# brade31919/radar_depth

Measured on AMD Instinct MI355X. Metric: training samples/sec, resnet18_latefusion b=16 450x800 rgbd, 1/2/4/8 MI355X, higher is better.
Workload: dtype f32

## Files before the change

include/radar_depth_hip.h:

```cpp
#ifndef RADAR_DEPTH_HIP_H
#define RADAR_DEPTH_HIP_H

#include <stdint.h>

#ifdef __cplusplus
extern "C" {
#endif

#define RD_OK 0
#define RD_EINVAL (-1)
#define RD_ELAUNCH (-2)

#define RD_MAX_TAPS 25
#define RD_MAX_PHASES 4

#define RD_ACT_NONE 0
#define RD_ACT_RELU 1
#define RD_ACT_LEAKY02 2

const char* rd_last_error(void);
int rd_abi_version(void);
int rd_device_info(int* n_cu, char* name, int name_len);

typedef struct {
    int32_t n_taps;
    int32_t out_off_h, out_off_w;
    int32_t lh, lw;
    int32_t dh_min, dh_max, dw_min, dw_max;
    int32_t tile_begin;
    int8_t dh[RD_MAX_TAPS];
    int8_t dw[RD_MAX_TAPS];
    int16_t widx[RD_MAX_TAPS];
} RdPhase;

typedef struct {
    int32_t N;
    int32_t Hi, Wi, Cin, ldi;
    int32_t Ho, Wo, Cout, ldo;
    int32_t in_stride, out_stride;
    int32_t n_phases;
    RdPhase phase[RD_MAX_PHASES];
} RdConvDesc;

int rd_gconv(const RdConvDesc* d, const float* in, const float* w_packed, float* out,
             const float* addend, int32_t ld_add, float* stat_partial, void* stream);
int rd_gconv_stat_tiles(const RdConvDesc* d);
int64_t rd_gconv_workspace_floats(const RdConvDesc* d);
int rd_gconv_stat_tiles_ws(const RdConvDesc* d);
int rd_gconv_ws(const RdConvDesc* d, const float* in, const float* w_packed, float* out,
                const float* addend, int32_t ld_add, float* stat_partial, float* ws, void* stream);
int rd_gconv_bnbwd_supported(const RdConvDesc* d);
int rd_gconv_bnbwd(const RdConvDesc* d, const float* dout, const float* w_packed, float* dx, const float* bn_x, int32_t ld_x,
                   const float* bn_mean, const float* bn_scale, const float* bn_shift, int32_t act, float* red_partial, float* ws,
                   void* stream);
int rd_gconv_fused(const RdConvDesc* d, const float* in, const float* w_packed, float* out, const float* bias,
                   int32_t act, int32_t act_cols, const float* addend, int32_t ld_add, float* ws, void* stream);
int rd_gconv_bf16(const RdConvDesc* d, const float* in, const void* w_packed_bf16, float* out, const float* bias,
                  int32_t act, int32_t act_cols, const float* addend, int32_t ld_add, float* stat_partial, void* stream);
int rd_gconv_bf16_stat_tiles(const RdConvDesc* d);
int rd_gconv_bf16_plan_info(const RdConvDesc* d, int32_t* out);
int rd_gconv_bf16_stat_tiles_t(int32_t dtype, const RdConvDesc* d);
int rd_gconv_bf16_plan_info_t(int32_t dtype, const RdConvDesc* d, int32_t* out);
int rd_gconv_bf16p_plan_all(int32_t on);
int rd_gconv_bf16_trace_read(unsigned long long* host, int n_wg);
int rd_gconv_split_supported(const RdConvDesc* d);
int rd_gconv_split_plan_all(int on);
int rd_gconv_split(const RdConvDesc* d, const float* in, const void* w_split, int64_t piece_elems, float* out, const float* bias,
                   int32_t act, int32_t act_cols, const float* addend, int32_t ld_add, float* stat_partial, void* stream);
int rd_gconv_split_stat_tiles(const RdConvDesc* d);
int rd_gconv_split_plan_info(const RdConvDesc* d, int32_t* out);
int rd_gemm_taps_split_supported(const RdConvDesc* d);
int rd_gemm_taps_split_preferred(const RdConvDesc* d);
int rd_gemm_taps_split_stat_tiles(const RdConvDesc* d);
int rd_gemm_taps_split_plan_info(const RdConvDesc* d, int32_t* out);
int rd_gemm_taps_split(const RdConvDesc* d, const float* in, const void* w_split, int64_t piece_elems, float* out, const float* bias,
                       int32_t act, int32_t act_cols, const float* addend, int32_t ld_add, float* stat_partial, void* stream);
int rd_split_pieces(const float* x, int32_t ldx, int64_t M, int32_t C, void* pieces, int64_t piece_elems, void* stream);
int rd_gconv_split_bnbwd_supported(const RdConvDesc* d, int32_t pre);
int rd_gconv_split_bnbwd(const RdConvDesc* d, const float* in, const void* w_split, int64_t piece_elems, float* out, const float* bn_x,
                         int32_t bn_ld, const float* mean, const float* scale, const float* shift, int32_t bn_act, float* red_partial, void* stream);
int rd_gconv_split_pre_bnbwd(const RdConvDesc* d, const void* in_pieces, int64_t in_piece_elems, const void* w_split, int64_t piece_elems,
                             float* out, const float* bn_x, int32_t bn_ld, const float* mean, const float* scale, const float* shift,
                             int32_t bn_act, float* red_partial, void* stream);
int rd_gconv_split_pre_supported(const RdConvDesc* d);
int rd_gconv_split_pre_preferred(const RdConvDesc* d);
int rd_gconv_split_pre(const RdConvDesc* d, const void* in_pieces, int64_t in_piece_elems, const void* w_split, int64_t piece_elems, float* out,
                       const float* bias, int32_t act, int32_t act_cols, const float* addend, int32_t ld_add, float* stat_partial, void* stream);
int rd_gconv_split_pre_stat_tiles(const RdConvDesc* d);
int rd_gconv_split_pre_plan_info(const RdConvDesc* d, int32_t* out);
int rd_gconv_split_slot_map(const RdConvDesc* d, int32_t pre, int32_t phase, int32_t* out, int32_t* slots, int32_t n_slots);
int rd_gconv_split_trace_read(unsigned long long* host, int n_wg);
int rd_wgrad_split_supported(const RdConvDesc* d);
int64_t rd_wgrad_split_workspace_floats(const RdConvDesc* d);
int rd_wgrad_split(const RdConvDesc* d, const float* in, const float* dout, float* slabs, void* stream);
int rd_wgrad_split_reduce(const RdConvDesc* d, const float* slabs, float* grad_oihw, int32_t O, int32_t I, int32_t KH, int32_t KW,
                          int32_t co_off, int32_t accumulate, void* stream);
int rd_wgrad_split_plan_info(const RdConvDesc* d, int32_t* out);
int rd_wgrad_split_pre_supported(const RdConvDesc* d);
int rd_wgrad_split_pre(const RdConvDesc* d, const void* x_pieces, int64_t x_piece_elems, const void* dy_pieces, int64_t dy_piece_elems,
                       float* slabs, void* stream);
int rd_gconv_plan_info(const RdConvDesc* d, int32_t* out);
int rd_gconv_occupancy(const RdConvDesc* d);
int rd_gconv_trace_read(unsigned long long* host, int n_wg);

int64_t rd_wgrad_workspace_floats(const RdConvDesc* d);
int rd_wgrad(const RdConvDesc* d, const float* in, const float* dout, float* slabs, void* stream);
int rd_wgrad_reduce(const RdConvDesc* d, const float* slabs, float* grad_oihw, int32_t O, int32_t I,
                    int32_t KH, int32_t KW, int32_t co_off, int32_t accumulate, void* stream);
int rd_wgrad_plan_info(const RdConvDesc* d, int32_t* out);

int rd_pack_weights(const float* w_oihw, float* packed, int32_t O, int32_t I, int32_t KH, int32_t KW,
                    int32_t ldc, int32_t co_off, int32_t rows_total, int32_t transpose, void* stream);

typedef struct {
    const float* slabs;
    float* tmp;
    float* grad;
    int64_t E;
    int32_t n_splits, J, S, Cin, Cout, O, I, co_off, accumulate;
    int32_t first_block1, n_blocks1, first_block2, n_blocks2;
    int32_t pad_;
} RdReduceJob;
int rd_wgrad_reduce_job(const RdConvDesc* d, int32_t bf16_kernel, const float* slabs, float* grad_oihw, int32_t O, int32_t I,
                        int32_t KH, int32_t KW, int32_t co_off, int32_t accumulate, RdReduceJob* job);
int rd_wgrad_reduce_batched(const RdReduceJob* jobs_dev, const int32_t* block_job1_dev, int32_t n_blocks1,
                            const int32_t* block_job2_dev, int32_t n_blocks2, void* stream);

int rd_wgrad_bf16_supported(const RdConvDesc* d);
int64_t rd_wgrad_bf16_workspace_floats(const RdConvDesc* d);
int rd_wgrad_bf16(const RdConvDesc* d, const float* in, const float* dout, float* slabs, void* stream);
int rd_wgrad_bf16_reduce(const RdConvDesc* d, const float* slabs, float* grad_oihw, int32_t O, int32_t I, int32_t KH,
                         int32_t KW, int32_t co_off, int32_t accumulate, void* stream);
int rd_wgrad_bf16_plan_info(const RdConvDesc* d, int32_t* out);
int rd_wgrad_bf16_trace_read(unsigned long long* host, int n_wg);

int rd_pack_weights_bf16(const float* w_oihw, void* packed_bf16, int32_t O, int32_t I, int32_t KH, int32_t KW,
                         int32_t ldc, int32_t co_off, int32_t rows_total, int32_t transpose, void* stream);

int rd_pack_chunk(void);
int rd_pack_weights_batched(const void* jobs_dev, const int32_t* block_job_dev, int32_t n_blocks, void* stream);

int rd_stem_fwd(const float* const* planes, const int64_t* strides, int32_t Cin, int32_t N, int32_t H,
                int32_t W, const float* w_packed, int32_t Cout, float* out, float* stat_partial,
                void* stream);
int rd_stem_stat_tiles(int32_t N, int32_t H, int32_t W);
int rd_stem_fwd_bf16(const float* const* planes, const int64_t* strides, int32_t Cin, int32_t N, int32_t H,
                     int32_t W, const float* w_packed, int32_t Cout, float* out, float* stat_partial,
                     void* stream);
int rd_stem_fwd_split(const float* const* planes, const int64_t* strides, int32_t Cin, int32_t N, int32_t H,
                      int32_t W, const float* w_packed, int32_t Cout, float* out, float* stat_partial,
                      void* stream);
int rd_conv16_split_supported(const RdConvDesc* d);
int rd_conv16_split(const RdConvDesc* d, const float* in, const float* w_packed, float* out, const float* addend, int32_t ld_add,
                    float* stat_partial, void* stream);
int64_t rd_stem_wgrad_workspace_floats(int32_t N, int32_t H, int32_t W, int32_t Cin, int32_t Cout);
int rd_stem_wgrad(const float* const* planes, const int64_t* strides, int32_t Cin, int32_t N, int32_t H,
                  int32_t W, const float* dout, int32_t Cout, float* grad_oihw, float* ws, void* stream);
int rd_stem_wgrad_split_supported(int32_t Cin, int32_t Cout);
int rd_stem_wgrad_split_t(int32_t dtype, const float* const* planes, const int64_t* strides, int32_t Cin, int32_t N, int32_t H,
                          int32_t W, const void* dout, int32_t Cout, float* grad_oihw, float* ws, void* stream);
int rd_stem_wgrad_split_bn_t(int32_t dtype, const float* const* planes, const int64_t* strides, int32_t Cin, int32_t N, int32_t H,
                             int32_t W, const void* g, const void* x, const float* red_partial, int32_t n_tiles, const float* gamma,
                             const float* mean, const float* invstd, float* dgamma, float* dbeta, float* coef_ws, int32_t Cout,
                             float* grad_oihw, float* ws, void* stream);
int rd_stem_dgrad_channel(const float* dout, const float* w_packed, int32_t N, int32_t H, int32_t W,
                          int32_t Cin, int32_t ci, int32_t Cout, float* dx, void* stream);

int rd_bn_finalize(const float* stat_partial, int32_t n_tiles, int32_t ld, int32_t c0, int32_t C, int64_t count,
                   const float* gamma, const float* beta, float eps, float momentum,
                   float* running_mean, float* running_var, int64_t* num_batches_tracked,
                   float* mean, float* invstd, float* scale, float* shift, void* stream);
int rd_bn_eval_coeffs(int32_t C, const float* gamma, const float* beta, const float* running_mean,
                      const float* running_var, float eps, float* scale, float* shift, void* stream);
int rd_bn_eval_coeffs_batched(const void* jobs_dev, int32_t n_jobs, float eps, void* stream);
int rd_bn_stats(const float* x, int64_t M, int32_t C, int32_t ldx, float* stat_partial, int32_t* n_tiles,
                void* stream);
int rd_bn_stats_tiles(int64_t M);
int rd_bn_act(const float* x1, int32_t ldx1, const float* scale1, const float* shift1,
              const float* x2, int32_t ldx2, const float* scale2, const float* shift2,
              float* y, int32_t ldy, int64_t M, int32_t C, int32_t act, void* stream);
int rd_bn_bwd_reduce(const float* dy, int32_t lddy, const float* y, int32_t ldy,
                     const float* x1, int32_t ldx1, const float* mean1,
                     const float* x2, int32_t ldx2, const float* mean2,
                     float* g, int32_t ldg, int64_t M, int32_t C, int32_t act,
                     float* red_partial, void* stream);
int rd_bn_bwd_reduce_x(const float* dy, int32_t lddy, const float* x1, int32_t ldx1, const float* mean1,
                       const float* scale1, const float* shift1, float* g, int32_t ldg, int64_t M, int32_t C,
                       int32_t act, float* red_partial, void* stream);
int rd_bn_bwd_tiles(int64_t M, int32_t C);
int rd_bn_bwd_apply(const float* g, int32_t ldg, const float* x, int32_t ldx, const float* red_partial,
                    int32_t n_tiles, int32_t which, const float* gamma, const float* mean,
                    const float* invstd, float* dgamma, float* dbeta, float* coef_ws ,
                    float* dx, int32_t lddx, int64_t M, int32_t C, void* stream);
int rd_bn_bwd_apply_x(const float* dy, int32_t lddy, const float* x, int32_t ldx, const float* red_partial, int32_t n_tiles,
                      const float* gamma, const float* mean, const float* invstd, const float* scale, const float* shift,
                      int32_t act, float* dgamma, float* dbeta, float* coef_ws, float* dx, int32_t lddx, int64_t M, int32_t C,
                      void* stream);
int rd_bn_bwd_reduce_x2(const float* dy, int32_t lddy, const float* x1, int32_t ldx1, const float* mean1, const float* scale1,
                        const float* shift1, const float* x2, int32_t ldx2, const float* mean2, const float* scale2,
                        const float* shift2, int64_t M, int32_t C, int32_t act, float* red_partial, void* stream);
int rd_bn_bwd_apply_x2(const float* dy, int32_t lddy, const float* x1, int32_t ldx1, const float* x2, int32_t ldx2,
                       const float* red_partial, int32_t n_tiles, const float* gamma1, const float* mean1, const float* invstd1,
                       const float* scale1, const float* shift1, const float* gamma2, const float* mean2, const float* invstd2,
                       const float* scale2, const float* shift2, int32_t act, float* dgamma1, float* dbeta1, float* dgamma2,
                       float* dbeta2, float* coef_ws6, float* dx1, int32_t lddx1, float* dx2, int32_t lddx2, int64_t M,
                       int32_t C, void* stream);

int rd_bnact_maxpool_fwd(const float* x, const float* scale, const float* shift, int32_t act,
                         int32_t N, int32_t H, int32_t W, int32_t C, float* y, int32_t ldy,
                         uint8_t* idx, void* stream);
int rd_bnact_maxpool_bwd(const float* dy, int32_t lddy, const uint8_t* idx, const float* x,
                         const float* scale, const float* shift, int32_t act, int32_t N, int32_t H,
                         int32_t W, int32_t C, float* g, void* stream);
int rd_bnact_maxpool_bwd_tiles(int32_t N, int32_t H, int32_t W, int32_t C);
int rd_bnact_maxpool_bwd_stats(const float* dy, int32_t lddy, const uint8_t* idx, const float* x, const float* scale,
                               const float* shift, int32_t act, int32_t N, int32_t H, int32_t W, int32_t C, float* g,
                               const float* mean, float* red_partial, void* stream);

int rd_head_conv_fwd(const float* x, int32_t ldx, const float* w_oihw, int32_t N, int32_t H, int32_t W,
                     int32_t C, float* d, void* stream);
int rd_head_conv_bwd(const float* x, int32_t ldx, const float* w_oihw, const float* dd, int32_t N,
                     int32_t H, int32_t W, int32_t C, float* dx, int32_t lddx, float* dw_oihw,
                     float* ws, void* stream);
int64_t rd_head_conv_bwd_workspace_floats(int32_t N, int32_t H, int32_t W, int32_t C);
int rd_bilinear_fwd(const float* d, int32_t N, int32_t Hs, int32_t Ws, float* out, int32_t Ho, int32_t Wo,
                    void* stream);
int rd_bilinear_bwd(const float* dout, int32_t N, int32_t Ho, int32_t Wo, float* dd, int32_t Hs, int32_t Ws,
                    void* stream);

int rd_masked_l1_sums(const float* pred, const float* target, int64_t n, float* ws, double* sums, void* stream);
int rd_loss_tiles(int64_t n);
int rd_masked_l1_bwd(const float* pred, const float* target, int64_t n, const double* sums,
                     const float* coef, float* dpred, int32_t accumulate, void* stream);
int rd_masked_l2_sums(const float* pred, const float* target, int64_t n, float* ws, double* sums, void* stream);
int rd_masked_l2_bwd(const float* pred, const float* target, int64_t n, const double* sums,
                     const float* coef, float* dpred, int32_t accumulate, void* stream);
int rd_depth_metrics(const float* output, const float* target, int64_t n, float* ws, double* sums, void* stream);
int rd_masked_l1_sums_metrics(const float* pred, const float* target, int64_t n, float* ws, double* sums,
                              double* msums, void* stream);
int rd_masked_l2_sums_metrics(const float* pred, const float* target, int64_t n, float* ws, double* sums,
                              double* msums, void* stream);
int64_t rd_depth_metrics_frames_workspace_floats(int32_t frames, int64_t hw);
int rd_depth_metrics_frames(const float* output, const float* target, int32_t frames, int64_t hw, float* ws,
                            double* sums, void* stream);
int rd_meter_update(const double* sums, int32_t rows, const double* weights, const int32_t* groups,
                    int32_t n_groups, double* meter, double* last, void* stream);
int64_t rd_smooth_workspace_floats(int32_t N, int32_t H, int32_t W);
int rd_smooth_fwd(const float* pred, const float* image, int32_t N, int32_t C, int32_t H, int32_t W,
                  float* ws, double* out, void* stream);
int rd_smooth_bwd(int32_t N, int32_t H, int32_t W, const float* ws, const float* coef, float* dpred,
// ... 163 lines not shown
```

radar_depth_amd/csrc/wgrad_split.hip:

```cpp
#include <math.h>
#include <stdlib.h>

#include <mutex>
#include <string>
#include <unordered_map>

#include "common.h"

namespace rd {

int launch_slab_reduce(const float* slabs, int n_splits, int64_t E, float* tmp, float* grad_oihw, int S, int Cin, int Cout,
                       int O, int I, int co_off, int accumulate, hipStream_t s);

typedef __bf16 wsbf16x8 __attribute__((ext_vector_type(8)));
typedef short wss16x4 __attribute__((ext_vector_type(4)));
typedef unsigned int wsu32x4 __attribute__((ext_vector_type(4)));
typedef float wsf32x2 __attribute__((ext_vector_type(2)));
typedef __bf16 wsbf16x2 __attribute__((ext_vector_type(2)));

constexpr unsigned WS_OOB = 0x80000000u;
template <int R_, int TW_>
struct WsGeo {
    static constexpr int R = R_, TW = TW_;
    static constexpr int XW = TW + 2, XH = R + 2;
    static constexpr int XPIX = XW * XH, YPIX = R * TW;
    static constexpr int XPLANE = ((XPIX * 64 + 255) / 256) * 256;
    static constexpr int YPLANE = YPIX * 64;
    static constexpr int XBYTES = 3 * 2 * XPLANE;
    static constexpr int YBYTES = 3 * 2 * YPLANE;
    static constexpr int BUF = XBYTES + YBYTES;
    static constexpr int XUNITS = XPIX * 8;
    static constexpr int XUNITS_PAD = ((XUNITS + 63) / 64) * 64;
    static constexpr int UNITS = XUNITS_PAD + YPIX * 8;
    static constexpr int UPT = (UNITS + 255) / 256;
    static_assert(YPIX == 64 && TW % 16 == 0, "a tile is 64 pixels in 16-pixel reduction steps");
    static constexpr int XP16 = ((XPIX * 32 + 127) / 256) * 256 + 128;
    static constexpr int YP16 = ((YPIX * 32 + 127) / 256) * 256 + 128;
    static constexpr int XBYTES_P = 3 * 4 * XP16;
    static constexpr int YBYTES_P = 3 * 4 * YP16;
    static constexpr int BUF_P = XBYTES_P + YBYTES_P;
    static constexpr int XSEG = (XW + 31) / 32, YSEG = (TW + 31) / 32;
    static constexpr int XU_P = 3 * 4 * XH * XSEG;
    static constexpr int YU_P = 3 * 4 * R * YSEG;
};
typedef WsGeo<2, 32> WsWide;
typedef WsGeo<4, 16> WsTall;

struct WsArgs {
    const float* x;
    const float* dy;
    float* slabs;
    int N, Hi, Wi, Cin, ldi, Ho, Wo, Cout, ldo;
    int tiles_h, tiles_w, total_tiles, tiles_per_split, n_splits, n_cib, n_cob;
    int dh0, dw0;
    int OS, off_h, off_w;
    int lh, lw;
    int S;
    int widx[9];
    const unsigned short* xp;
    const unsigned short* yp;
    long long xplane, yplane;
    long long xm, ym;
    int dbg;
};

__device__ __forceinline__ unsigned ws_cvt_pk(float a, float b) {
    wsf32x2 v;
    v[0] = a; v[1] = b;
    return __builtin_bit_cast(unsigned, __builtin_convertvector(v, wsbf16x2));
}
__device__ __forceinline__ void ws_split8(const float4 v0, const float4 v1, wsu32x4& w0, wsu32x4& w1, wsu32x4& w2) {
    const float x[8] = {v0.x, v0.y, v0.z, v0.w, v1.x, v1.y, v1.z, v1.w};
#pragma unroll
    for (int i = 0; i < 4; ++i) {
        float a = x[2 * i], b = x[2 * i + 1];
        const unsigned u0 = ws_cvt_pk(a, b);
        a -= __uint_as_float(u0 << 16);
        b -= __uint_as_float(u0 & 0xffff0000u);
        const unsigned u1 = ws_cvt_pk(a, b);
        a -= __uint_as_float(u1 << 16);
        b -= __uint_as_float(u1 & 0xffff0000u);
        w0[i] = u0;
        w1[i] = u1;
        w2[i] = ws_cvt_pk(a, b);
    }
}

template <int PITCH = 64>
__device__ __forceinline__ wsbf16x8 ws_frag(unsigned base, int off) {
    typedef __attribute__((address_space(3))) wss16x4* lp;
    const wss16x4 lo = __builtin_amdgcn_ds_read_tr16_b64_v4i16(reinterpret_cast<lp>(base + off));
    const wss16x4 hi = __builtin_amdgcn_ds_read_tr16_b64_v4i16(reinterpret_cast<lp>(base + off + 4 * PITCH));
    typedef short s16x8 __attribute__((ext_vector_type(8)));
    s16x8 r;
    r[0] = lo[0]; r[1] = lo[1]; r[2] = lo[2]; r[3] = lo[3];
    r[4] = hi[0]; r[5] = hi[1]; r[6] = hi[2]; r[7] = hi[3];
    return __builtin_bit_cast(wsbf16x8, r);
}

template <int TR, int TC, typename G, bool PRE>
__global__ __launch_bounds__(512) void wgrad_split_kernel(const WsArgs a) {
    constexpr int NT = TR * TC;
    constexpr int BUFB = PRE ? G::BUF_P : G::BUF;
    constexpr int PIT = PRE ? 32 : 64;
    extern __shared__ __attribute__((aligned(16))) float smem[];
    const int tid = threadIdx.x, lane = tid & 63;
    const int wave = __builtin_amdgcn_readfirstlane(tid >> 6);
    const bool loader = wave >= 4;
    const unsigned lds0 = (unsigned)(size_t)smem;

    const int vid = xcd_remap(blockIdx.x, gridDim.x);
    const int nblk = a.n_cib * a.n_cob;
    const int blk = vid % nblk, split = vid / nblk;
    const int cib0 = (blk / a.n_cob) * 64, cob0 = (blk % a.n_cob) * 64;
    const int tile_begin = split * a.tiles_per_split;
    const int tile_end = min(tile_begin + a.tiles_per_split, a.total_tiles);
    const int ntiles = tile_end - tile_begin;

    f32x16 acc[NT];

    if (loader && PRE) {
        const int lw = wave - 4;
        const char* xsrc = reinterpret_cast<const char*>(a.xp);
        const char* ysrc = reinterpret_cast<const char*>(a.yp);
        const int pxl = lane >> 1, hf = lane & 1;
        auto stage = [&](int tile, int buf) {
            const int n = tile / (a.tiles_h * a.tiles_w), tr = tile - n * (a.tiles_h * a.tiles_w);
            const int r0 = (tr / a.tiles_w) * G::R, c0 = (tr % a.tiles_w) * G::TW;
            const unsigned base = lds0 + buf * BUFB;
            for (int u = lw; u < G::XU_P + G::YU_P; u += 4) {
                if (u < G::XU_P) {
                    const int sg = u % G::XSEG, u1 = u / G::XSEG;
                    const int row = u1 % G::XH, t = u1 / G::XH, blk = t & 3, p = t >> 2;
                    const int px = sg * 32 + pxl;
                    const int ih = r0 + a.dh0 + row, iw = c0 + a.dw0 + px, ch = cib0 + blk * 16;
                    const bool rok = ih >= 0 && ih < a.Hi && ch < a.Cin;
                    const bool ok = rok && px < G::XW && iw >= 0 && iw < a.Wi;
                    const unsigned dst = base + (p * 4 + blk) * G::XP16 + (row * G::XW + sg * 32) * 32;
                    if (ok) glds16(reinterpret_cast<const float*>(xsrc + p * a.xplane + (((size_t)(ch >> 4) * a.xm + ((size_t)n * a.Hi + ih) * a.Wi + iw) * 32 + hf * 16)),
                                   reinterpret_cast<float*>((size_t)dst));
                    else if (px < G::XW) asm volatile("ds_write_b128 %0, %1" ::"v"(dst + lane * 16), "v"(wsu32x4{0u, 0u, 0u, 0u}) : "memory");
                } else {
                    const int v = u - G::XU_P;
                    const int sg = v % G::YSEG, v1 = v / G::YSEG;
                    const int row = v1 % G::R, t = v1 / G::R, blk = t & 3, p = t >> 2;
                    const int px = sg * 32 + pxl;
                    const int lr = r0 + row, lc = c0 + px, ch = cob0 + blk * 16;
                    const int oh = a.OS * lr + a.off_h, ow = a.OS * lc + a.off_w;
                    const bool ok = lr < a.lh && ch < a.Cout && px < G::TW && lc < a.lw;
                    const unsigned dst = base + G::XBYTES_P + (p * 4 + blk) * G::YP16 + (row * G::TW + sg * 32) * 32;
                    if (ok) glds16(reinterpret_cast<const float*>(ysrc + p * a.yplane + (((size_t)(ch >> 4) * a.ym + ((size_t)n * a.Ho + oh) * a.Wo + ow) * 32 + hf * 16)),
                                   reinterpret_cast<float*>((size_t)dst));
                    else if (px < G::TW) asm volatile("ds_write_b128 %0, %1" ::"v"(dst + lane * 16), "v"(wsu32x4{0u, 0u, 0u, 0u}) : "memory");
                }
            }
        };
        if (ntiles > 0) stage(tile_begin, 0);
        glds_wait();
        for (int i = 0; i < ntiles; ++i) {
            rd_sync();
            if (i + 1 < ntiles) stage(tile_begin + i + 1, (i + 1) & 1);
            glds_wait();
        }
        rd_sync();
    } else if (loader) {
        const int ltid = tid - 256;
        int upr[G::UPT], upc[G::UPT], uch[G::UPT], udst[G::UPT];
#pragma unroll
        for (int u = 0; u < G::UPT; ++u) {
            const int e = ltid + 256 * u;
            if (e < G::XUNITS) {
                const int t = e / (G::XPIX * 4), rem = e - t * (G::XPIX * 4);
                const int px = rem >> 2, q = rem & 3;
                upr[u] = px / G::XW; upc[u] = px - upr[u] * G::XW;
                uch[u] = t * 32 + q * 8;
                udst[u] = t * G::XPLANE + rem * 16;
            } else if (e >= G::XUNITS_PAD && e < G::UNITS) {
                const int e2 = e - G::XUNITS_PAD;
                const int t = e2 >> 8, rem = e2 & 255;
                const int px = rem >> 2, q = rem & 3;
                upr[u] = px / G::TW; upc[u] = px - upr[u] * G::TW;
                uch[u] = t * 32 + q * 8;
                udst[u] = G::XBYTES + t * G::YPLANE + rem * 16;
            } else {
                upr[u] = upc[u] = uch[u] = 0;
                udst[u] = -1;
            }
        }
        const unsigned ximg = (unsigned)(a.Hi * a.Wi * a.ldi) * 4u, yimg = (unsigned)(a.Ho * a.Wo * a.ldo) * 4u;
        float4 va0[G::UPT], va1[G::UPT], vb0[G::UPT], vb1[G::UPT];
        auto fetch = [&](int tile, float4 (&v0)[G::UPT], float4 (&v1)[G::UPT]) {
            if (a.dbg & 4) return;
            const int n = tile / (a.tiles_h * a.tiles_w), tr = tile - n * (a.tiles_h * a.tiles_w);
            const int r0 = (tr / a.tiles_w) * G::R, c0 = (tr % a.tiles_w) * G::TW;
            const __amdgpu_buffer_rsrc_t rx = __builtin_amdgcn_make_buffer_rsrc(const_cast<float*>(a.x) + (size_t)n * a.Hi * a.Wi * a.ldi, 0, ximg, 0x00020000);
            const __amdgpu_buffer_rsrc_t ry = __builtin_amdgcn_make_buffer_rsrc(const_cast<float*>(a.dy) + (size_t)n * a.Ho * a.Wo * a.ldo, 0, yimg, 0x00020000);
#pragma unroll
            for (int u = 0; u < G::UPT; ++u) {
                const bool is_x = __builtin_amdgcn_readfirstlane(ltid + 256 * u) < G::XUNITS_PAD;
                unsigned off;
                if (is_x) {
                    const int ih = r0 + a.dh0 + upr[u], iw = c0 + a.dw0 + upc[u], ch = cib0 + uch[u];
                    off = (ih >= 0 && ih < a.Hi && iw >= 0 && iw < a.Wi && ch < a.Cin && udst[u] >= 0) ? (unsigned)(((ih * a.Wi + iw) * a.ldi + ch) * 4) : WS_OOB;
                    v0[u] = __builtin_bit_cast(float4, __builtin_amdgcn_raw_buffer_load_b128(rx, (int)off, 0, 0));
                    v1[u] = __builtin_bit_cast(float4, __builtin_amdgcn_raw_buffer_load_b128(rx, (int)off + 16, 0, 0));
                } else {
                    const int lr = r0 + upr[u], lc = c0 + upc[u], ch = cob0 + uch[u];
                    const int oh = a.OS * lr + a.off_h, ow = a.OS * lc + a.off_w;
                    off = (lr < a.lh && lc < a.lw && ch < a.Cout && udst[u] >= 0) ? (unsigned)(((oh * a.Wo + ow) * a.ldo + ch) * 4) : WS_OOB;
                    v0[u] = __builtin_bit_cast(float4, __builtin_amdgcn_raw_buffer_load_b128(ry, (int)off, 0, 0));
                    v1[u] = __builtin_bit_cast(float4, __builtin_amdgcn_raw_buffer_load_b128(ry, (int)off + 16, 0, 0));
                }
            }
        };
        auto split_put = [&](int buf, float4 (&v0)[G::UPT], float4 (&v1)[G::UPT]) {
            const unsigned base = lds0 + buf * BUFB;
#pragma unroll
            for (int u = 0; u < G::UPT; ++u) {
                wsu32x4 w0, w1, w2;
                if (a.dbg & 1) { w0 = __builtin_bit_cast(wsu32x4, v0[u]); w1 = __builtin_bit_cast(wsu32x4, v1[u]); w2 = w0; }
                else ws_split8(v0[u], v1[u], w0, w1, w2);
                if (udst[u] >= 0 && !(a.dbg & 2)) {
                    const bool is_x = udst[u] < G::XBYTES;
                    const unsigned pstride = is_x ? 2 * G::XPLANE : 2 * G::YPLANE;
                    const unsigned ad = base + udst[u];
                    asm volatile("ds_write_b128 %0, %1" ::"v"(ad), "v"(w0) : "memory");
                    asm volatile("ds_write_b128 %0, %1" ::"v"(ad + pstride), "v"(w1) : "memory");
                    asm volatile("ds_write_b128 %0, %1" ::"v"(ad + 2 * pstride), "v"(w2) : "memory");
                }
                __builtin_amdgcn_sched_barrier(0);
            }
        };
        if (ntiles > 0) {
            fetch(tile_begin, va0, va1);
            if (ntiles > 1) fetch(tile_begin + 1, vb0, vb1);
            split_put(0, va0, va1);
        }
        asm volatile("s_waitcnt lgkmcnt(0)" ::: "memory");
        for (int i = 0; i < ntiles; i += 2) {
            rd_sync();
            if (i + 2 < ntiles) fetch(tile_begin + i + 2, va0, va1);
            if (i + 1 < ntiles) split_put(1, vb0, vb1);
            asm volatile("s_waitcnt lgkmcnt(0)" ::: "memory");
            if (i + 1 >= ntiles) break;
            rd_sync();
            if (i + 3 < ntiles) fetch(tile_begin + i + 3, vb0, vb1);
            if (i + 2 < ntiles) split_put(0, va0, va1);
            asm volatile("s_waitcnt lgkmcnt(0)" ::: "memory");
        }
        rd_sync();
    } else {
#pragma unroll
        for (int t = 0; t < NT; ++t)
#pragma unroll
            for (int i = 0; i < 16; ++i) acc[t][i] = 0.f;
        const int ti = wave >> 1, to = wave & 1;
        const unsigned lrow = (unsigned)(((lane & 15) >> 2) + (lane >> 5) * 8) * PIT + (lane & 3) * 8;
        const unsigned xb = PRE ? lds0 + (2 * ti + ((lane >> 4) & 1)) * G::XP16 + lrow : lds0 + ti * G::XPLANE + lrow + ((lane >> 4) & 1) * 32;
        const unsigned yb = PRE ? lds0 + G::XBYTES_P + (2 * to + ((lane >> 4) & 1)) * G::YP16 + lrow : lds0 + G::XBYTES + to * G::YPLANE + lrow + ((lane >> 4) & 1) * 32;
        constexpr int XPS = PRE ? 4 * G::XP16 : 2 * G::XPLANE;
        constexpr int YPS = PRE ? 4 * G::YP16 : 2 * G::YPLANE;
        for (int i = 0; i < ntiles; ++i) {
            rd_sync();
            const unsigned xa = xb + (i & 1) * BUFB, ya = yb + (i & 1) * BUFB;
            constexpr int NSTEP = G::R * (G::TW / 16) * NT;
            wsbf16x8 A[2][3], B[2][3];
            auto loadA = [&](int s_, wsbf16x8 (&F)[3]) {
                const int rk = s_ / NT, t = s_ % NT, r = rk / (G::TW / 16), ks = rk % (G::TW / 16);
#pragma unroll
                for (int p = 0; p < 3; ++p) F[p] = ws_frag<PIT>(xa, p * XPS + ((r + t / TC) * G::XW + ks * 16 + t % TC) * PIT);
            };
            auto loadB = [&](int rk, wsbf16x8 (&F)[3]) {
                const int r = rk / (G::TW / 16), ks = rk % (G::TW / 16);
#pragma unroll
                for (int p = 0; p < 3; ++p) F[p] = ws_frag<PIT>(ya, p * YPS + (r * G::TW + ks * 16) * PIT);
            };
            loadB(0, B[0]);
            loadA(0, A[0]);
#pragma unroll
            for (int s_ = 0; s_ < NSTEP; ++s_) {
                const int rk = s_ / NT, t = s_ % NT;
                if (s_ + 1 < NSTEP) {
                    loadA(s_ + 1, A[(s_ + 1) & 1]);
                    if (t == NT - 1) loadB(rk + 1, B[(rk + 1) & 1]);
                }
                __builtin_amdgcn_sched_barrier(0);
                f32x16 c = acc[t];
                RD_SPLIT_TERMS(c, A[s_ & 1][0], A[s_ & 1][1], A[s_ & 1][2], B[rk & 1][0], B[rk & 1][1], B[rk & 1][2])
                acc[t] = c;
                __builtin_amdgcn_sched_barrier(0);
            }
        }
        rd_sync();
        const int l31 = lane & 31, hh = lane >> 5;
        float* slab = a.slabs + (size_t)split * a.S * a.Cin * a.Cout;
        const int co = cob0 + to * 32 + l31;
#pragma unroll
        for (int t = 0; t < NT; ++t) {
            float* dst = slab + (size_t)a.widx[t] * a.Cin * a.Cout;
#pragma unroll
            for (int i = 0; i < 16; ++i) {
                const int ci = cib0 + ti * 32 + (i & 3) + 8 * (i >> 2) + 4 * hh;
                if (ci < a.Cin && co < a.Cout) dst[(size_t)ci * a.Cout + co] = acc[t][i];
            }
        }
    }
}

struct WsPlan {
    int ok, tiles_h, tiles_w, total_tiles, tiles_per_split, n_splits, n_cib, n_cob, J, S;
    int tall;
};

static bool ws_phase_ok(const RdPhase& p, int& tr, int& tc) {
    tr = p.dh_max - p.dh_min + 1;
    tc = p.dw_max - p.dw_min + 1;
    if (tr < 2 || tr > 3 || tc < 2 || tc > 3 || p.n_taps != tr * tc) return false;
    for (int t = 0; t < p.n_taps; ++t)
        if (p.dh[t] != p.dh_min + t / tc || p.dw[t] != p.dw_min + t % tc || p.widx[t] < 0) return false;
    return true;
}

static bool ws_shape_ok(const RdConvDesc& d) {
    static const char* off = getenv("RD_WGRAD_NO_SPLIT");
    if (off) return false;
    if (d.n_phases < 1 || d.n_phases > RD_MAX_PHASES || d.in_stride != 1 || d.out_stride < 1 || d.out_stride > 2) return false;
    if (d.n_phases == 1 && d.out_stride != 1) return false;
    if (d.n_phases > 1 && d.out_stride != 2) return false;
    for (int i = 0; i < d.n_phases; ++i) {
        const RdPhase& p = d.phase[i];
        int tr, tc;
        if (!ws_phase_ok(p, tr, tc)) return false;
        if (p.lh != d.phase[0].lh || p.lw != d.phase[0].lw || p.lh > d.Hi || p.lw > d.Wi) return false;
        if (d.out_stride * (p.lh - 1) + p.out_off_h >= d.Ho || d.out_stride * (p.lw - 1) + p.out_off_w >= d.Wo) return false;
    }
    if (d.n_phases == 1 && d.phase[0].n_taps != 9) return false;
    if (d.Cin < 64 || d.Cout < 64 || d.Cin % 8 != 0 || d.Cout % 8 != 0 || d.ldi % 4 != 0 || d.ldo % 4 != 0) return false;
    if ((int64_t)d.Hi * d.Wi * d.ldi * 4 >= (int64_t)WS_OOB || (int64_t)d.Ho * d.Wo * d.ldo * 4 >= (int64_t)WS_OOB) return false;
    return true;
}

static WsPlan ws_plan(const RdConvDesc& d) {
    WsPlan pl{};
    pl.ok = ws_shape_ok(d) ? 1 : 0;
    if (!pl.ok) return pl;
    {
        const int lh = d.phase[0].lh, lw = d.phase[0].lw;
        const long long wide_px = (long long)cdiv(lh, WsWide::R) * WsWide::R * cdiv(lw, WsWide::TW) * WsWide::TW;
        const long long tall_px = (long long)cdiv(lh, WsTall::R) * WsTall::R * cdiv(lw, WsTall::TW) * WsTall::TW;
        static const char* force = getenv("RD_WGRAD_SPLIT_TILE");
        pl.tall = force ? (force[0] == 't') : (tall_px * 10 <= wide_px * 11);
        pl.tiles_h = cdiv(lh, pl.tall ? WsTall::R : WsWide::R);
        pl.tiles_w = cdiv(lw, pl.tall ? WsTall::TW : WsWide::TW);
    }
    pl.total_tiles = d.N * pl.tiles_h * pl.tiles_w;
    pl.n_cib = cdiv(d.Cin, 64);
    pl.n_cob = cdiv(d.Cout, 64);
    for (int i = 0; i < d.n_phases; ++i)
        for (int t = 0; t < d.phase[i].n_taps; ++t) pl.S = pl.S > d.phase[i].widx[t] + 1 ? pl.S : d.phase[i].widx[t] + 1;
    static const char* wpc = getenv("RD_WGRAD_SPLIT_WG_PER_CU");
    int ns = (wpc ? atoi(wpc) : 1) * num_cus() / (pl.n_cib * pl.n_cob);
    if (ns < 1) ns = 1;
    const int max_ns = cdiv(pl.total_tiles, 4);
    if (ns > max_ns) ns = max_ns < 1 ? 1 : max_ns;
    pl.tiles_per_split = cdiv(pl.total_tiles, ns);
    pl.n_splits = cdiv(pl.total_tiles, pl.tiles_per_split);
    pl.J = pl.n_splits < 16 ? pl.n_splits : 16;
    return pl;
}

template <int TR, int TC, typename G, bool PRE>
static int launch_ws(const WsArgs& a, int grid, hipStream_t s) {
    static std::atomic<unsigned long long> attr_set{0};
    auto k = wgrad_split_kernel<TR, TC, G, PRE>;
    RD_SET_ATTR_ONCE(attr_set, hipFuncSetAttribute(reinterpret_cast<const void*>(k), hipFuncAttributeMaxDynamicSharedMemorySize, 160 * 1024));
    hipLaunchKernelGGL(k, dim3(grid), dim3(512), 2 * (PRE ? G::BUF_P : G::BUF), s, a);
    RD_CHECK_LAUNCH("wgrad_split_kernel");
    return RD_OK;
}

}

using namespace rd;

extern "C" int rd_wgrad_split_supported(const RdConvDesc* d) { return d && ws_shape_ok(*d) ? 1 : 0; }

extern "C" int64_t rd_wgrad_split_workspace_floats(const RdConvDesc* d) {
    if (!d) return RD_EINVAL;
    const WsPlan pl = ws_plan(*d);
    if (!pl.ok) return RD_EINVAL;
    return (int64_t)(pl.n_splits + pl.J) * pl.S * d->Cin * d->Cout;
}

extern "C" int rd_wgrad_split_plan_info(const RdConvDesc* d, int32_t* out) {
    if (!d || !out) return RD_EINVAL;
    const WsPlan pl = ws_plan(*d);
    if (!pl.ok) return RD_EINVAL;
    out[0] = pl.n_splits; out[1] = pl.tiles_per_split; out[2] = pl.n_splits * pl.n_cib * pl.n_cob; out[3] = pl.total_tiles + (pl.tall ? 1 << 30 : 0);
    return RD_OK;
}

template <bool PRE>
static int ws_launch_all(const RdConvDesc* d, WsArgs& a, const WsPlan& pl, hipStream_t s) {
    const int grid = pl.n_splits * pl.n_cib * pl.n_cob;
    for (int i = 0; i < d->n_phases; ++i) {
        const RdPhase& p = d->phase[i];
        int tr, tc;
        ws_phase_ok(p, tr, tc);
        a.dh0 = p.dh_min; a.dw0 = p.dw_min; a.off_h = p.out_off_h; a.off_w = p.out_off_w; a.lh = p.lh; a.lw = p.lw;
        for (int t = 0; t < 9; ++t) a.widx[t] = t < p.n_taps ? p.widx[t] : 0;
        int rc;
        if (pl.tall) {
            if (tr == 3 && tc == 3) rc = launch_ws<3, 3, WsTall, PRE>(a, grid, s);
            else if (tr == 2 && tc == 3) rc = launch_ws<2, 3, WsTall, PRE>(a, grid, s);
            else if (tr == 3 && tc == 2) rc = launch_ws<3, 2, WsTall, PRE>(a, grid, s);
            else rc = launch_ws<2, 2, WsTall, PRE>(a, grid, s);
        } else {
            if (tr == 3 && tc == 3) rc = launch_ws<3, 3, WsWide, PRE>(a, grid, s);
            else if (tr == 2 && tc == 3) rc = launch_ws<2, 3, WsWide, PRE>(a, grid, s);
            else if (tr == 3 && tc == 2) rc = launch_ws<3, 2, WsWide, PRE>(a, grid, s);
            else rc = launch_ws<2, 2, WsWide, PRE>(a, grid, s);
        }
        if (rc != RD_OK) return rc;
    }
    return RD_OK;
}

static void ws_fill_args(const RdConvDesc* d, const WsPlan& pl, WsArgs& a) {
    a.N = d->N; a.Hi = d->Hi; a.Wi = d->Wi; a.Cin = d->Cin; a.ldi = d->ldi; a.Ho = d->Ho; a.Wo = d->Wo; a.Cout = d->Cout; a.ldo = d->ldo;
    a.tiles_h = pl.tiles_h; a.tiles_w = pl.tiles_w; a.total_tiles = pl.total_tiles; a.tiles_per_split = pl.tiles_per_split;
    a.n_splits = pl.n_splits; a.n_cib = pl.n_cib; a.n_cob = pl.n_cob;
    a.OS = d->out_stride; a.S = pl.S;
    a.x = nullptr; a.dy = nullptr; a.xp = nullptr; a.yp = nullptr; a.xplane = a.yplane = 0;
    { const char* dbg = getenv("RD_WGRAD_SPLIT_DEBUG"); a.dbg = dbg ? atoi(dbg) : 0; }
    a.xm = (long long)d->N * d->Hi * d->Wi; a.ym = (long long)d->N * d->Ho * d->Wo;
}

extern "C" int rd_wgrad_split(const RdConvDesc* d, const float* in, const float* dout, float* slabs, void* stream) {
    RD_CHECK_ARG(d && in && dout && slabs, "wgrad_split: null argument");
    const WsPlan pl = ws_plan(*d);
    if (!pl.ok) { set_error("wgrad_split: descriptor not supported (rd_wgrad_split_supported)"); return RD_EINVAL; }
    RD_CHECK_ARG(reinterpret_cast<uintptr_t>(in) % 16 == 0 && reinterpret_cast<uintptr_t>(dout) % 16 == 0, "wgrad_split: unaligned tensor");
    WsArgs a;
    ws_fill_args(d, pl, a);
    a.x = in; a.dy = dout; a.slabs = slabs;
    return ws_launch_all<false>(d, a, pl, static_cast<hipStream_t>(stream));
}

extern "C" int rd_wgrad_split_pre_supported(const RdConvDesc* d) { return d && ws_shape_ok(*d) && d->Cin % 16 == 0 && d->Cout % 16 == 0 ? 1 : 0; }

extern "C" int rd_wgrad_split_pre(const RdConvDesc* d, const void* x_pieces, int64_t x_piece_elems, const void* dy_pieces, int64_t dy_piece_elems,
                                  float* slabs, void* stream) {
    RD_CHECK_ARG(d && x_pieces && dy_pieces && slabs, "wgrad_split_pre: null argument");
    const WsPlan pl = ws_plan(*d);
    if (!pl.ok || d->Cin % 16 || d->Cout % 16) { set_error("wgrad_split_pre: descriptor not supported (rd_wgrad_split_pre_supported)"); return RD_EINVAL; }
    RD_CHECK_ARG(reinterpret_cast<uintptr_t>(x_pieces) % 16 == 0 && reinterpret_cast<uintptr_t>(dy_pieces) % 16 == 0, "wgrad_split_pre: unaligned tensor");
    WsArgs a;
    ws_fill_args(d, pl, a);
    RD_CHECK_ARG(x_piece_elems >= (int64_t)d->Cin * a.xm && dy_piece_elems >= (int64_t)d->Cout * a.ym && x_piece_elems % 8 == 0 && dy_piece_elems % 8 == 0,
                 "wgrad_split_pre: piece stride too small");
    a.xp = static_cast<const unsigned short*>(x_pieces); a.yp = static_cast<const unsigned short*>(dy_pieces);
    a.xplane = (long long)x_piece_elems * 2; a.yplane = (long long)dy_piece_elems * 2;
    a.slabs = slabs;
    return ws_launch_all<true>(d, a, pl, static_cast<hipStream_t>(stream));
}

extern "C" int rd_wgrad_split_reduce(const RdConvDesc* d, const float* slabs, float* grad_oihw, int32_t O, int32_t I, int32_t KH, int32_t KW,
                                     int32_t co_off, int32_t accumulate, void* stream) {
    RD_CHECK_ARG(d && slabs && grad_oihw, "wgrad_split_reduce: null argument");
    const WsPlan pl = ws_plan(*d);
    if (!pl.ok) { set_error("wgrad_split_reduce: descriptor not supported"); return RD_EINVAL; }
    RD_CHECK_ARG(KH * KW == pl.S && I == d->Cin && co_off >= 0 && co_off + O <= d->Cout, "wgrad_split_reduce: gradient shape does not match the descriptor");
    const int64_t E = (int64_t)pl.S * d->Cin * d->Cout;
    float* tmp = const_cast<float*>(slabs) + (int64_t)pl.n_splits * E;
    return launch_slab_reduce(slabs, pl.n_splits, E, tmp, grad_oihw, pl.S, d->Cin, d->Cout, O, I, co_off, accumulate, static_cast<hipStream_t>(stream));
}
```

radar_depth_amd/ops.py:

```python
import ctypes as C
import os as _os

import torch

from . import _lib
from ._lib import check, current_stream, lib, ptr


def _f32(t):
    assert t.dtype == torch.float32 and t.is_cuda and t.is_contiguous(), "expected contiguous CUDA float32 tensor"
    return t


def pack_weights(w_oihw, transpose=False, out=None, ldc=None, off=0, rows_total=None):
    o, i, kh, kw = w_oihw.shape
    if not transpose:
        ldc = ldc or o
        rows_total = i
        shape = (kh * kw, i, ldc)
    else:
        ldc = ldc or i
        rows_total = rows_total or o
        shape = (kh * kw, rows_total, ldc)
    if out is None:
# ... 83 lines not shown
                                   ptr(_f32(out)), ptr(bias), act, act_cols, ptr(addend), ld_add, ptr(stat), current_stream()), "rd_gconv_split_pre")
    return out


def gconv_split_pre_stat_tiles(desc):
    n = lib().rd_gconv_split_pre_stat_tiles(C.byref(desc))
    if n < 0:
        check(n, "rd_gconv_split_pre_stat_tiles")
    return n


def gconv_split_stat_tiles(desc):
    n = lib().rd_gconv_split_stat_tiles(C.byref(desc))
    if n < 0:
        check(n, "rd_gconv_split_stat_tiles")
    return n


def gconv_stat_tiles(desc):
    n = lib().rd_gconv_stat_tiles_ws(C.byref(desc))
    if n < 0:
        check(n, "rd_gconv_stat_tiles_ws")
    return n


_WS = {}


def _poison():
    if _os.environ.get("RD_POISON_LDS") == "1":
        check(lib().rd_debug_poison_lds(current_stream()), "rd_debug_poison_lds")


def gconv(desc, x, w_packed, out, addend=None, ld_add=0, stat=None):
    _poison()
    n = int(lib().rd_gconv_workspace_floats(C.byref(desc)))
    if n < 0:
        check(n, "rd_gconv_workspace_floats")
    ws = None
    if n > 0:
        ws = _WS.get((n, out.device))
        if ws is None:
            ws = _WS[(n, out.device)] = torch.empty(n, dtype=torch.float32, device=out.device)
    check(lib().rd_gconv_ws(C.byref(desc), ptr(x), ptr(w_packed), ptr(out), ptr(addend), ld_add, ptr(stat), ptr(ws),
                            current_stream()), "rd_gconv_ws")
    return out


def gconv_bnbwd(desc, dout, w_packed, dx, bn_x, ld_x, mean, scale, shift, act, red):
    _poison()
    check(lib().rd_gconv_bnbwd(C.byref(desc), ptr(dout), ptr(w_packed), ptr(dx), ptr(bn_x), ld_x, ptr(mean), ptr(scale), ptr(shift),
                               act, ptr(red), None, current_stream()), "rd_gconv_bnbwd")
    return dx


def fill(t, v):
    check(lib().rd_fill(ptr(t), C.c_int64(t.numel()), C.c_float(v), current_stream()), "rd_fill")
    return t


def nchw_to_nhwc(x):
    n, c, h, w = x.shape
    out = torch.empty((n, h, w, c), dtype=torch.float32, device=x.device)
    check(lib().rd_nchw_to_nhwc(ptr(_f32(x)), ptr(out), n, c, h, w, current_stream()), "rd_nchw_to_nhwc")
    return out


def nhwc_to_nchw(x):
    n, h, w, c = x.shape
    out = torch.empty((n, c, h, w), dtype=torch.float32, device=x.device)
    check(lib().rd_nhwc_to_nchw(ptr(_f32(x)), ptr(out), n, c, h, w, current_stream()), "rd_nhwc_to_nchw")
    return out


def wgrad_workspace_floats(desc):
    n = lib().rd_wgrad_workspace_floats(C.byref(desc))
    if n < 0:
        check(int(n), "rd_wgrad_workspace_floats")
    return int(n)


def wgrad(desc, x, dout, slabs):
    _poison()
    check(lib().rd_wgrad(C.byref(desc), ptr(x), ptr(dout), ptr(slabs), current_stream()), "rd_wgrad")
    return slabs


def wgrad_reduce(desc, slabs, grad_oihw, co_off=0, accumulate=False):
    o, i, kh, kw = grad_oihw.shape
    check(lib().rd_wgrad_reduce(C.byref(desc), ptr(slabs), ptr(_f32(grad_oihw)), o, i, kh, kw, co_off, int(accumulate),
                                current_stream()), "rd_wgrad_reduce")
    return grad_oihw


def wgrad_reduce_batched(jobs):
    import numpy as np
    from ._lib import RdReduceJob
    arr = (RdReduceJob * len(jobs))()
    bj1, bj2 = [], []
    for q, (desc, slabs, grad, co_off) in enumerate(jobs):
        o, i, kh, kw = grad.shape
        check(lib().rd_wgrad_reduce_job(C.byref(desc), 0, ptr(slabs), ptr(_f32(grad)), o, i, kh, kw, co_off, 0, C.byref(arr[q])), "rd_wgrad_reduce_job")
        arr[q].first_block1, arr[q].first_block2 = len(bj1), len(bj2)
        bj1 += [q] * arr[q].n_blocks1
        bj2 += [q] * arr[q].n_blocks2
    dev = jobs[0][1].device
    table = torch.from_numpy(np.frombuffer(bytes(arr), dtype=np.uint8).copy()).to(dev)
    t1 = torch.tensor(bj1 or [0], dtype=torch.int32, device=dev)
    t2 = torch.tensor(bj2, dtype=torch.int32, device=dev)
    check(lib().rd_wgrad_reduce_batched(ptr(table), ptr(t1), len(bj1), ptr(t2), len(bj2), current_stream()), "rd_wgrad_reduce_batched")
    torch.cuda.current_stream().synchronize()
    return len(bj1), len(bj2)


def bn_stats(x2d, C_):
    M = x2d.shape[0]
    tiles = lib().rd_bn_stats_tiles(C.c_int64(M))
    part = torch.zeros(tiles, 2, C_, device=x2d.device)
    nt = C.c_int32(0)
    check(lib().rd_bn_stats(ptr(x2d), C.c_int64(M), C_, x2d.stride(0), ptr(part), C.byref(nt), current_stream()), "rd_bn_stats")
    assert nt.value == tiles
    return part, tiles


def wgrad_bf16(desc, x, dout, grad_oihw):
    _poison()
    n = int(lib().rd_wgrad_bf16_workspace_floats(C.byref(desc)))
    if n < 0:
        check(n, "rd_wgrad_bf16_workspace_floats")
    slabs = torch.empty(n, dtype=torch.float32, device=x.device)
    check(lib().rd_wgrad_bf16(C.byref(desc), ptr(_f32(x)), ptr(_f32(dout)), ptr(slabs), current_stream()), "rd_wgrad_bf16")
    o, i, kh, kw = grad_oihw.shape
    check(lib().rd_wgrad_bf16_reduce(C.byref(desc), ptr(slabs), ptr(_f32(grad_oihw)), o, i, kh, kw, 0, 0, current_stream()),
          "rd_wgrad_bf16_reduce")
    return grad_oihw


def wgrad_split_supported(desc):
    return lib().rd_wgrad_split_supported(C.byref(desc)) == 1


def wgrad_split_workspace_floats(desc):
    n = int(lib().rd_wgrad_split_workspace_floats(C.byref(desc)))
    if n < 0:
        check(n, "rd_wgrad_split_workspace_floats")
    return n


def wgrad_split(desc, x, dout, slabs):
    _poison()
    check(lib().rd_wgrad_split(C.byref(desc), ptr(_f32(x)), ptr(_f32(dout)), ptr(slabs), current_stream()), "rd_wgrad_split")


def wgrad_split_pre_supported(desc):
    return lib().rd_wgrad_split_pre_supported(C.byref(desc)) == 1


def wgrad_split_pre(desc, x_pieces, dy_pieces, slabs):
    _poison()
    check(lib().rd_wgrad_split_pre(C.byref(desc), ptr(x_pieces), C.c_int64(x_pieces[0].numel()), ptr(dy_pieces), C.c_int64(dy_pieces[0].numel()),
                                   ptr(slabs), current_stream()), "rd_wgrad_split_pre")


def wgrad_split_reduce(desc, slabs, grad, co_off=0, accumulate=False):
    o, i, kh, kw = grad.shape
    check(lib().rd_wgrad_split_reduce(C.byref(desc), ptr(slabs), ptr(grad), o, i, kh, kw, co_off, int(accumulate), current_stream()),
          "rd_wgrad_split_reduce")


def wino_supported(H, W, cin, cout, ldi=None, ldo=None):
    return lib().rd_wino_supported(H, W, cin, cout, cin if ldi is None else ldi, cout if ldo is None else ldo) == 1


def wino_pack(w_oihw, flip=False):
    o, i, kh, kw = w_oihw.shape
    assert kh == 3 and kw == 3
    lib().rd_wino_packed_bytes.restype = C.c_int64
    nbytes = int(lib().rd_wino_packed_bytes(o, i, int(flip)))
    u = torch.empty(nbytes // 2, dtype=torch.bfloat16, device=w_oihw.device)
    check(lib().rd_wino_pack(ptr(_f32(w_oihw.contiguous())), o, i, int(flip), ptr(u), current_stream()), "rd_wino_pack")
    return u


def wino_conv3x3(x_nhwc, u_packed, out_nhwc, addend=None, stat=None):
    n, h, w, cin = x_nhwc.shape
    cout = out_nhwc.shape[3]
    for t in (x_nhwc, out_nhwc) + ((addend,) if addend is not None else ()):
        assert t.dtype == torch.float32 and t.is_cuda and t.stride(3) == 1 and t.stride(1) == t.shape[2] * t.stride(2) and t.stride(0) == t.shape[1] * t.stride(1), \
            "expected an NHWC CUDA float32 tensor (a channel slice of a wider buffer is fine)"
    check(lib().rd_wino_conv3x3(ptr(x_nhwc), n, h, w, cin, x_nhwc.stride(2), ptr(u_packed), ptr(out_nhwc), cout, out_nhwc.stride(2),
                                ptr(addend), 0 if addend is None else addend.stride(2), ptr(stat), current_stream()), "rd_wino_conv3x3")
    return out_nhwc


def wino_stat_tiles(n, h, w):
    return int(lib().rd_wino_stat_tiles(n, h, w))
```

Baseline: 1063.

## Skip out-of-range K-steps in tall wgrad tiles and re-cost tile choice by steps

For the tall tile geometry (R=4, TW=16), the wgrad-split MFMA loop now reorders its K dimension into quads of 4 pixels along the row. It bounds the number of K-steps per tile by the valid width of that tile column, so partial right-edge tiles skip MFMA work on padding. The tall-versus-wide tile heuristic now compares MFMA step counts instead of padded pixel counts. The change also adds a step_info query and Python helpers. The risks are more register pressure and branching in the inner loop, and a possible correctness issue in the new LDS fragment addressing.

New measurement: 1073, median of 6. No clear change (+0.9%).

```diff
diff --git a/include/radar_depth_hip.h b/include/radar_depth_hip.h
--- a/include/radar_depth_hip.h
+++ b/include/radar_depth_hip.h
@@ -96,6 +96,7 @@
 int rd_wgrad_split_reduce(const RdConvDesc* d, const float* slabs, float* grad_oihw, int32_t O, int32_t I, int32_t KH, int32_t KW,
                           int32_t co_off, int32_t accumulate, void* stream);
 int rd_wgrad_split_plan_info(const RdConvDesc* d, int32_t* out);
+int rd_wgrad_split_step_info(const RdConvDesc* d, int32_t out[4]);
 int rd_wgrad_split_pre_supported(const RdConvDesc* d);
 int rd_wgrad_split_pre(const RdConvDesc* d, const void* x_pieces, int64_t x_piece_elems, const void* dy_pieces, int64_t dy_piece_elems,
                        float* slabs, void* stream);
diff --git a/radar_depth_amd/csrc/wgrad_split.hip b/radar_depth_amd/csrc/wgrad_split.hip
--- a/radar_depth_amd/csrc/wgrad_split.hip
+++ b/radar_depth_amd/csrc/wgrad_split.hip
@@ -86,16 +86,13 @@
     }
 }
 
-template <int PITCH = 64>
-__device__ __forceinline__ wsbf16x8 ws_frag(unsigned base, int off) {
+template <int HI>
+__device__ __forceinline__ wsu32x4 ws_frag(unsigned base, int off) {
     typedef __attribute__((address_space(3))) wss16x4* lp;
-    const wss16x4 lo = __builtin_amdgcn_ds_read_tr16_b64_v4i16(reinterpret_cast<lp>(base + off));
-    const wss16x4 hi = __builtin_amdgcn_ds_read_tr16_b64_v4i16(reinterpret_cast<lp>(base + off + 4 * PITCH));
-    typedef short s16x8 __attribute__((ext_vector_type(8)));
-    s16x8 r;
-    r[0] = lo[0]; r[1] = lo[1]; r[2] = lo[2]; r[3] = lo[3];
-    r[4] = hi[0]; r[5] = hi[1]; r[6] = hi[2]; r[7] = hi[3];
-    return __builtin_bit_cast(wsbf16x8, r);
+    typedef unsigned int u32x2 __attribute__((ext_vector_type(2)));
+    const u32x2 lo = __builtin_bit_cast(u32x2, __builtin_amdgcn_ds_read_tr16_b64_v4i16(reinterpret_cast<lp>(base + off)));
+    const u32x2 hi = __builtin_bit_cast(u32x2, __builtin_amdgcn_ds_read_tr16_b64_v4i16(reinterpret_cast<lp>(base + off + HI)));
+    return wsu32x4{lo[0], lo[1], hi[0], hi[1]};
 }
 
 template <int TR, int TC, typename G, bool PRE>
@@ -255,40 +252,53 @@
 #pragma unroll
             for (int i = 0; i < 16; ++i) acc[t][i] = 0.f;
         const int ti = wave >> 1, to = wave & 1;
-        const unsigned lrow = (unsigned)(((lane & 15) >> 2) + (lane >> 5) * 8) * PIT + (lane & 3) * 8;
-        const unsigned xb = PRE ? lds0 + (2 * ti + ((lane >> 4) & 1)) * G::XP16 + lrow : lds0 + ti * G::XPLANE + lrow + ((lane >> 4) & 1) * 32;
-        const unsigned yb = PRE ? lds0 + G::XBYTES_P + (2 * to + ((lane >> 4) & 1)) * G::YP16 + lrow : lds0 + G::XBYTES + to * G::YPLANE + lrow + ((lane >> 4) & 1) * 32;
+        constexpr bool QS = G::R == 4 && G::TW == 16;
+        constexpr int XQ = QS ? G::XW : 4, YQ = QS ? G::TW : 4;
+        constexpr int NK = G::R * (G::TW / 16);
+        auto lrow = [&](int quad) { return (unsigned)(((lane & 15) >> 2) + (lane >> 5) * 2 * quad) * PIT + (lane & 3) * 8; };
+        const unsigned xb = PRE ? lds0 + (2 * ti + ((lane >> 4) & 1)) * G::XP16 + lrow(XQ) : lds0 + ti * G::XPLANE + lrow(XQ) + ((lane >> 4) & 1) * 32;
+        const unsigned yb = PRE ? lds0 + G::XBYTES_P + (2 * to + ((lane >> 4) & 1)) * G::YP16 + lrow(YQ) : lds0 + G::XBYTES + to * G::YPLANE + lrow(YQ) + ((lane >> 4) & 1) * 32;
         constexpr int XPS = PRE ? 4 * G::XP16 : 2 * G::XPLANE;
         constexpr int YPS = PRE ? 4 * G::YP16 : 2 * G::YPLANE;
+        int ct = tile_begin % a.tiles_w;
         for (int i = 0; i < ntiles; ++i) {
+            const int nq = QS ? min(NK, (a.lw - ct * G::TW + 3) >> 2) : NK;
+            ct = ct + 1 == a.tiles_w ? 0 : ct + 1;
             rd_sync();
             const unsigned xa = xb + (i & 1) * BUFB, ya = yb + (i & 1) * BUFB;
-            constexpr int NSTEP = G::R * (G::TW / 16) * NT;
-            wsbf16x8 A[2][3], B[2][3];
-            auto loadA = [&](int s_, wsbf16x8 (&F)[3]) {
-                const int rk = s_ / NT, t = s_ % NT, r = rk / (G::TW / 16), ks = rk % (G::TW / 16);
-#pragma unroll
-                for (int p = 0; p < 3; ++p) F[p] = ws_frag<PIT>(xa, p * XPS + ((r + t / TC) * G::XW + ks * 16 + t % TC) * PIT);
+            wsu32x4 A[2][3], B[2][3];
+            auto loadA = [&](int s_, wsu32x4 (&F)[3]) {
+                const int rk = s_ / NT, t = s_ % NT;
+                const int px = QS ? (t / TC) * G::XW + rk * 4 + t % TC : (rk / (G::TW / 16) + t / TC) * G::XW + rk % (G::TW / 16) * 16 + t % TC;
+#pragma unroll
+                for (int p = 0; p < 3; ++p) F[p] = ws_frag<XQ * PIT>(xa, p * XPS + px * PIT);
             };
-            auto loadB = [&](int rk, wsbf16x8 (&F)[3]) {
-                const int r = rk / (G::TW / 16), ks = rk % (G::TW / 16);
-#pragma unroll
-                for (int p = 0; p < 3; ++p) F[p] = ws_frag<PIT>(ya, p * YPS + (r * G::TW + ks * 16) * PIT);
+            auto loadB = [&](int rk, wsu32x4 (&F)[3]) {
+                const int px = QS ? rk * 4 : rk / (G::TW / 16) * G::TW + rk % (G::TW / 16) * 16;
+#pragma unroll
+                for (int p = 0; p < 3; ++p) F[p] = ws_frag<YQ * PIT>(ya, p * YPS + px * PIT);
             };
             loadB(0, B[0]);
             loadA(0, A[0]);
 #pragma unroll
-            for (int s_ = 0; s_ < NSTEP; ++s_) {
-                const int rk = s_ / NT, t = s_ % NT;
-                if (s_ + 1 < NSTEP) {
-                    loadA(s_ + 1, A[(s_ + 1) & 1]);
-                    if (t == NT - 1) loadB(rk + 1, B[(rk + 1) & 1]);
+            for (int rk = 0; rk < NK; ++rk) {
+                if (rk < nq) {
+#pragma unroll
+                    for (int t = 0; t < NT; ++t) {
+                        const int s_ = rk * NT + t;
+                        if (t + 1 < NT) loadA(s_ + 1, A[(s_ + 1) & 1]);
+                        else if (rk + 1 < NK && rk + 1 < nq) {
+                            loadA(s_ + 1, A[(s_ + 1) & 1]);
+                            loadB(rk + 1, B[(rk + 1) & 1]);
+                        }
+                        __builtin_amdgcn_sched_barrier(0);
+                        f32x16 c = acc[t];
+                        auto fr = [](const wsu32x4 v) { return __builtin_bit_cast(wsbf16x8, v); };
+                        RD_SPLIT_TERMS(c, fr(A[s_ & 1][0]), fr(A[s_ & 1][1]), fr(A[s_ & 1][2]), fr(B[rk & 1][0]), fr(B[rk & 1][1]), fr(B[rk & 1][2]))
+                        acc[t] = c;
+                        __builtin_amdgcn_sched_barrier(0);
+                    }
                 }
-                __builtin_amdgcn_sched_barrier(0);
-                f32x16 c = acc[t];
-                RD_SPLIT_TERMS(c, A[s_ & 1][0], A[s_ & 1][1], A[s_ & 1][2], B[rk & 1][0], B[rk & 1][1], B[rk & 1][2])
-                acc[t] = c;
-                __builtin_amdgcn_sched_barrier(0);
             }
         }
         rd_sync();
@@ -310,6 +320,7 @@
 struct WsPlan {
     int ok, tiles_h, tiles_w, total_tiles, tiles_per_split, n_splits, n_cib, n_cob, J, S;
     int tall;
+    int steps_wide, steps_tall;
 };
 
 static bool ws_phase_ok(const RdPhase& p, int& tr, int& tc) {
@@ -346,10 +357,10 @@
     if (!pl.ok) return pl;
     {
         const int lh = d.phase[0].lh, lw = d.phase[0].lw;
-        const long long wide_px = (long long)cdiv(lh, WsWide::R) * WsWide::R * cdiv(lw, WsWide::TW) * WsWide::TW;
-        const long long tall_px = (long long)cdiv(lh, WsTall::R) * WsTall::R * cdiv(lw, WsTall::TW) * WsTall::TW;
+        pl.steps_wide = cdiv(lh, WsWide::R) * cdiv(lw, WsWide::TW) * 4;
+        pl.steps_tall = cdiv(lh, WsTall::R) * cdiv(lw, 4);
         static const char* force = getenv("RD_WGRAD_SPLIT_TILE");
-        pl.tall = force ? (force[0] == 't') : (tall_px * 10 <= wide_px * 11);
+        pl.tall = force ? (force[0] == 't') : ((long long)pl.steps_tall * 10 <= (long long)pl.steps_wide * 11);
         pl.tiles_h = cdiv(lh, pl.tall ? WsTall::R : WsWide::R);
         pl.tiles_w = cdiv(lw, pl.tall ? WsTall::TW : WsWide::TW);
     }
@@ -397,6 +408,18 @@
     const WsPlan pl = ws_plan(*d);
     if (!pl.ok) return RD_EINVAL;
     out[0] = pl.n_splits; out[1] = pl.tiles_per_split; out[2] = pl.n_splits * pl.n_cib * pl.n_cob; out[3] = pl.total_tiles + (pl.tall ? 1 << 30 : 0);
+    return RD_OK;
+}
+
+extern "C" int rd_wgrad_split_step_info(const RdConvDesc* d, int32_t* out) {
+    if (!d || !out) return RD_EINVAL;
+    const WsPlan pl = ws_plan(*d);
+    if (!pl.ok) return RD_EINVAL;
+    const int lh = d->phase[0].lh, lw = d->phase[0].lw;
+    out[0] = pl.tall ? pl.steps_tall : pl.steps_wide;
+    out[1] = pl.tall ? cdiv(lh, WsTall::R) * cdiv(lw, WsTall::TW) * 4 : pl.steps_wide;
+    out[2] = (int32_t)cdiv64((int64_t)lh * lw, 16);
+    out[3] = pl.tall;
     return RD_OK;
 }
 
diff --git a/radar_depth_amd/ops.py b/radar_depth_amd/ops.py
--- a/radar_depth_amd/ops.py
+++ b/radar_depth_amd/ops.py
@@ -259,6 +259,18 @@
     check(lib().rd_wgrad_split(C.byref(desc), ptr(_f32(x)), ptr(_f32(dout)), ptr(slabs), current_stream()), "rd_wgrad_split")
 
 
+def wgrad_split_plan_info(desc):
+    v = (C.c_int32 * 4)()
+    check(lib().rd_wgrad_split_plan_info(C.byref(desc), v), "rd_wgrad_split_plan_info")
+    return v[0], v[1], v[2], v[3] & ((1 << 30) - 1), bool(v[3] >> 30)
+
+
+def wgrad_split_step_info(desc):
+    v = (C.c_int32 * 4)()
+    check(lib().rd_wgrad_split_step_info(C.byref(desc), v), "rd_wgrad_split_step_info")
+    return v[0], v[1], v[2], bool(v[3])
+
+
 def wgrad_split_pre_supported(desc):
     return lib().rd_wgrad_split_pre_supported(C.byref(desc)) == 1
 
```
